# BIT-DYN/OpenObj

Measured on AMD Instinct MI355X. Metric: training rays/sec/GPU @64 samples/ray, 50 obj; PSNR delta vs ref, higher is better.
Workload: dtype f32; 1 GPU; c2: Replica room_0-shaped, 50 object MLPs on this GPU (hidden 32), 4096 rays/object/step, 64 samples/ray (16+48), RGB+depth+opacity loss, fused fwd+loss+bwd+AdamW; objects_per_gpu=50, objects_total=50, rays_per_object=4096, samples_per_ray=64, hidden=32, feature_head=False, background_mlp=True, parallelism=objects sharded x1, rccl_ranks=1, launched_by=single process, loss_status=0

## Files before the change

openobj_amd/csrc/objnerf_mlp32.h:

```cpp
#pragma once
#include "objnerf_mlp.h"

namespace obj32n {
using namespace obj32;

constexpr int WROW = 40;
constexpr int R_IN = 0;
constexpr int R_M1 = R_IN + 96;
constexpr int R_CAT = R_M1 + 32;
constexpr int R_M2 = R_CAT + 128;
constexpr int R_CL = R_M2 + 32;
constexpr int R_FL = R_CL + 80;
constexpr int ROWS_NOFEAT = R_FL, ROWS_FEAT = R_FL + 80;
constexpr int SV_BM1 = 0, SV_BM2 = 32, SV_WA = 64, SV_WOC = 96, SV_HB = 192, SV_PEB = 196, SV_FLOATS = 196 + 72 + 4;
__host__ __device__ constexpr int img_floats(bool feat) { return (feat ? ROWS_FEAT : ROWS_NOFEAT) * WROW + SV_FLOATS; }
__host__ __device__ constexpr int sv_base(bool feat) { return (feat ? ROWS_FEAT : ROWS_NOFEAT) * WROW; }

constexpr int BIAS_COL = -2, ZERO_COL = -1;
__host__ __device__ inline int x1_col(int t, int g) {
  const int i = t >> 2, f = t & 3, j = 4 * i + g;
  if (j < OBJ_NDIR) return 3 + OBJ_NDIR * f + j;
  if (f == 0) return g - 1;
  if (f == 1 && g == 1) return BIAS_COL;
  return ZERO_COL;
// ... 262 lines not shown
#pragma unroll
    for (int r = 0; r < 4; ++r) {
      const int col = x2_col(4 * T + r, g);
      e.x2[T][r] = col >= 0 ? emb[OBJ_E1 + col] : (col == BIAS_COL ? 1.0f : 0.0f);
    }
}

#ifdef OBJ_PRIO_TOGGLE
__device__ __forceinline__ void prio_layer(const int layer) {
  const int grp = __builtin_amdgcn_readfirstlane((int)(threadIdx.x >> 8)) & 1;
  if (layer >= 0 && ((layer ^ grp) & 1)) __builtin_amdgcn_s_setprio(1); else __builtin_amdgcn_s_setprio(0);
}
#else
__device__ __forceinline__ void prio_layer(const int) {}
#endif

template <bool FEAT>
__device__ __forceinline__ void mlp32_trunk(const float* wf, const float* sv, const int g, const Emb32& e, Acts& a) {
  T32 acc = zero32();
  prio_layer(1);
#pragma unroll
  for (int T = 0; T < 6; ++T) mma_f16(acc, wf, R_IN + 16 * T, e.x1[T]);
  a.h1 = relu32(acc);
  prio_layer(2);
#pragma unroll
  for (int tt = 0; tt < 2; ++tt)
#pragma unroll
    for (int r = 0; r < 4; ++r) acc.t[tt][r] = sv[SV_BM1 + 16 * tt + 4 * g + r];
  mma_f32(acc, wf, R_M1, a.h1);
  a.h2 = relu32(acc);
  prio_layer(3);
  acc = zero32();
  mma_f32(acc, wf, R_CAT, a.h2);
#pragma unroll
  for (int T = 0; T < 6; ++T) mma_f16(acc, wf, R_CAT + 32 + 16 * T, e.x1[T]);
  a.h3 = relu32(acc);
  prio_layer(4);
#pragma unroll
  for (int tt = 0; tt < 2; ++tt)
#pragma unroll
    for (int r = 0; r < 4; ++r) acc.t[tt][r] = sv[SV_BM2 + 16 * tt + 4 * g + r];
  mma_f32(acc, wf, R_M2, a.h3);
  a.h4 = relu32(acc);
  prio_layer(5);
  acc = zero32();
  mma_f32(acc, wf, R_CL, a.h4);
#pragma unroll
  for (int T = 0; T < 3; ++T) mma_f16(acc, wf, R_CL + 32 + 16 * T, e.x2[T]);
  a.hc = relu32(acc);
  if (FEAT) {
    acc = zero32();
    mma_f32(acc, wf, R_FL, a.h4);
#pragma unroll
    for (int T = 0; T < 3; ++T) mma_f16(acc, wf, R_FL + 32 + 16 * T, e.x2[T]);
    a.hf = relu32(acc);
  }
  prio_layer(-1);
}
__device__ __forceinline__ void mlp32_head_sums(const float* sv, const int g, const Acts& a, float& sa, float& s0, float& s1,
                                                float& s2) {
  float pa = 0.f, pc0 = 0.f, pc1 = 0.f, pc2 = 0.f;
#pragma unroll
  for (int tt = 0; tt < 2; ++tt)
#pragma unroll
    for (int r = 0; r < 4; ++r) {
      const int row = 16 * tt + 4 * g + r;
      pa = fmaf(sv[SV_WA + row], a.h4.t[tt][r], pa);
      pc0 = fmaf(sv[SV_WOC + row], a.hc.t[tt][r], pc0);
      pc1 = fmaf(sv[SV_WOC + H + row], a.hc.t[tt][r], pc1);
      pc2 = fmaf(sv[SV_WOC + 2 * H + row], a.hc.t[tt][r], pc2);
    }
  sa = xgroup_sum(pa); s0 = xgroup_sum(pc0); s1 = xgroup_sum(pc1); s2 = xgroup_sum(pc2);
}
template <bool FEAT>
__device__ __forceinline__ float mlp32_forward(const float* wf, const float* sv, const int g, const Emb32& e, Acts& a) {
  mlp32_trunk<FEAT>(wf, sv, g, e, a);
  float sa, s0, s1, s2;
  mlp32_head_sums(sv, g, a, sa, s0, s1, s2);
  const float mine = (g == 0) ? sa : ((g == 1) ? s0 : ((g == 2) ? s1 : s2));
  const float z = mine + sv[SV_HB + g];
  return (g == 0) ? z * 10.0f : sigmoid_acc(z);
}
template <bool FEAT>
__device__ __forceinline__ void mlp32_forward_all(const float* wf, const float* sv, const int g, const Emb32& e, Acts& a,
                                                  float& alpha10, float& colour) {
  mlp32_trunk<FEAT>(wf, sv, g, e, a);
  float sa, s0, s1, s2;
  mlp32_head_sums(sv, g, a, sa, s0, s1, s2);
  alpha10 = (sa + sv[SV_HB]) * 10.0f;
  const float mine = (g == 1) ? s0 : ((g == 2) ? s1 : s2);
  colour = (g == 0) ? 0.0f : sigmoid_acc(mine + sv[SV_HB + g]);
}

}
```

openobj_amd/csrc/objnerf_train32.hip:

```cpp
#include <mutex>
#include "objnerf_mlp32.h"
#include "objnerf_train_common.h"
#include "../../include/objnerf_hip.h"

using namespace obj32n;
using namespace objtrain;

#if !defined(OBJ_LAZY_HEADS) && !defined(OBJ_BUTTERFLY_HEADS)
#define OBJ_LAZY_HEADS
#endif

#ifndef OBJ32_ABL
#define OBJ32_ABL 0
#endif
#define TILE_SYNC() do { if (!((OBJ32_ABL) & 2)) __syncthreads(); } while (0)
#ifndef OBJ32_WG_UNROLL_FAST
#define OBJ32_WG_UNROLL_FAST 16
#endif

namespace {

__device__ __forceinline__ void st_T32(float* stg_lane, const int rowbase, const T32& v) {
  if ((OBJ32_ABL) & 4) { asm volatile("" :: "v"(v.t[0]), "v"(v.t[1])); return; }
#pragma unroll
// ... 23 lines not shown
    acc1 = OBJ_MFMA(a1[1], b[1], acc1);
  }
}

template <int UNR = 8>
__device__ __forceinline__ void wg_half(f32x4& acc0, const float* dT, const float* aT) {
  if ((OBJ32_ABL) & 8) return;
  dT = (const float*)__builtin_assume_aligned(dT, 8);
  aT = (const float*)__builtin_assume_aligned(aT, 8);
#pragma unroll UNR
  for (int st = 0; st < 32; st += 2) {
    const f32x2 b = *reinterpret_cast<const f32x2*>(aT + st);
    const f32x2 a0 = *reinterpret_cast<const f32x2*>(dT + st);
    acc0 = OBJ_MFMA(a0[0], b[0], acc0);
    acc0 = OBJ_MFMA(a0[1], b[1], acc0);
  }
}

template <int UNR = 8>
__device__ __forceinline__ void wg_quarter(f32x4& acc0, const float* dT, const float* aT, const int st0) {
  if ((OBJ32_ABL) & 8) return;
  dT = (const float*)__builtin_assume_aligned(dT, 8);
  aT = (const float*)__builtin_assume_aligned(aT, 8);
#pragma unroll UNR
  for (int st = st0; st < st0 + 16; st += 2) {
    const f32x2 b = *reinterpret_cast<const f32x2*>(aT + st);
    const f32x2 a0 = *reinterpret_cast<const f32x2*>(dT + st);
    acc0 = OBJ_MFMA(a0[0], b[0], acc0);
    acc0 = OBJ_MFMA(a0[1], b[1], acc0);
  }
}

__device__ __forceinline__ void wr_pair(float* slab, const f32x4& a0, const f32x4& a1, const int g, const int col,
                                        const int w_off, const int ncols, const int b_off) {
#pragma unroll
  for (int r = 0; r < 4; ++r) {
    const int o0 = 4 * g + r, o1 = 16 + 4 * g + r;
    if (col >= 0) {
      slab[w_off + o0 * ncols + col] = a0[r];
      slab[w_off + o1 * ncols + col] = a1[r];
    } else if (col == BIAS_COL && b_off >= 0) {
      slab[b_off + o0] = a0[r];
      slab[b_off + o1] = a1[r];
    }
  }
}

__device__ __forceinline__ void wr_half(float* slab, const f32x4& a0, const int half, const int g, const int col,
                                        const int w_off, const int ncols, const int b_off) {
#pragma unroll
  for (int r = 0; r < 4; ++r) {
    const int o = 16 * half + 4 * g + r;
    if (col >= 0) slab[w_off + o * ncols + col] = a0[r];
    else if (col == BIAS_COL && b_off >= 0) slab[b_off + o] = a0[r];
  }
}

#ifdef PHASE_TIMING
__device__ unsigned long long g_phase32[8][24];
#define PT_INIT() unsigned long long pt_acc[18]; for (int i_ = 0; i_ < 18; ++i_) pt_acc[i_] = 0; \
  unsigned long long pt_t0 = __builtin_amdgcn_s_memtime()
#define PT(i) do { const unsigned long long t_ = __builtin_amdgcn_s_memtime(); pt_acc[i] += t_ - pt_t0; pt_t0 = t_; } while (0)
#define PT_FLUSH() do { if (blockIdx.x == 0 && lane == 0) for (int i_ = 0; i_ < 18; ++i_) g_phase32[w][i_] = pt_acc[i_]; } while (0)
#else
#define PT_INIT() do {} while (0)
#define PT(i) do {} while (0)
#define PT_FLUSH() do {} while (0)
#endif

template <bool FEAT>
struct Lay {
  static constexpr int IMG = img_floats(FEAT);
  static constexpr int ROWS = FEAT ? 160 : STG_ROWS;
  static constexpr int LDS_FLOATS = IMG + SM_FLOATS + ROWS * STG_LD;
  static constexpr int A_H3 = FEAT ? 0 : 96, A_DHC = FEAT ? 80 : 128, A_DHF = 112, A_DH4 = FEAT ? 80 : 160;
  static constexpr int C_DH2 = FEAT ? 128 : 160;
  static_assert(LDS_FLOATS * 4 <= 163840, "LDS budget");
  static_assert((IMG * 4) % 16 == 0, "staging area alignment");
};
constexpr int F_SW = 144 * STG_LD;
constexpr int F_GFH = F_SW + TS;
constexpr int F_GOF = F_GFH + 16 * 32;
static_assert(F_GOF + 32 <= 160 * STG_LD && OFF_FHB + 64 * NWAVE <= 80 * STG_LD, "feature aliases");

template <bool FEAT, bool MASKS, int SS>
__global__ __launch_bounds__(NTHR) void train_fused32_kernel(const TrainDev a) {
  typedef Lay<FEAT> LY;
  constexpr int IMG = LY::IMG;
  constexpr bool FAST = !FEAT;
  constexpr int WGU = (!FEAT && !MASKS && SS == 64) ? OBJ32_WG_UNROLL_FAST : 8;
  extern __shared__ __attribute__((aligned(16))) float lds[];
  const int tid = threadIdx.x;
  const int lane = tid & 63;
  const int w = __builtin_amdgcn_readfirstlane(tid >> 6);
  const int c = lane & 15, g = lane >> 4;
  float* sv = lds + sv_base(FEAT);
  float* s_alpha = lds + IMG;
  float* s_col = s_alpha + TS;
  float* stg = lds + IMG + SM_FLOATS;

  const long T_flat = (long)a.K * a.NT;
  long cur = a.flat_nwg ? T_flat * blockIdx.x / a.flat_nwg : 0;
  const long cur_end = a.flat_nwg ? T_flat * (blockIdx.x + 1) / a.flat_nwg : 1;
  bool first_seg = true;
  while (cur < cur_end) {
  int k, t0, t1, tstep, sslot;
  if (a.flat_nwg) {
    k = (int)(cur / a.NT);
    t0 = (int)(cur - (long)k * a.NT);
    const long rem = cur_end - cur;
    t1 = (long)t0 + rem < (long)a.NT ? (int)(t0 + rem) : a.NT;
    tstep = 1;
    sslot = (int)blockIdx.x - flat_wg_of(T_flat, a.flat_nwg, (long)k * a.NT);
    cur += t1 - t0;
  } else {
    k = blockIdx.x / a.G; t0 = blockIdx.x % a.G; t1 = a.NT; tstep = a.G; sslot = t0;
    cur = cur_end;
  }
  const int n_slots = a.flat_nwg ? a.Gs : a.G;
  if (!first_seg) __syncthreads();
  first_seg = false;

  stage_weights32(lds, a.params + (long)k * a.p_stride, a.L, FEAT, tid, NTHR);
  for (int i = tid; i < LY::ROWS * STG_LD; i += NTHR) stg[i] = 0.0f;
  __syncthreads();

  const float scale = a.scale[k];
  const int S = SS ? SS : a.S, R = a.R, TR = SS ? TS / SS : a.TR;
  const float n1 = (float)a.counts[2 * k], n2 = (float)a.counts[2 * k + 1];
  int bflag0, bflag1;
  batch_flags(a, bflag0, bflag1);
  const float inv1 = bflag0 ? 0.0f : 1.0f / (n1 + 1e-10f);
  const float inv2 = bflag1 ? 0.0f : 1.0f / (n2 + 1e-10f);

  const float* wf = (const float*)__builtin_assume_aligned(lds + 4 * g * WROW + out_pos(c), 8);
  const float* wt0 = (const float*)__builtin_assume_aligned(lds + c * WROW + 8 * g + 4 * (g & 1), 16);
  const float* wt1 = (const float*)__builtin_assume_aligned(lds + c * WROW + 8 * g + 4 * (1 - (g & 1)), 16);
  float* stg_lane = stg + (4 * g) * STG_LD + 16 * w + c;
  const float* lane_rd = stg + c * STG_LD + 32 * g;

  f32x4 accA0 = zero4(), accA1 = zero4(), accB0 = zero4(), accB1 = zero4(), accC0 = zero4(), accC1 = zero4();
  f32x4 accA2 = zero4(), accC2 = zero4();
#ifdef OBJ_LAZY_HEADS
  constexpr bool LAZY_H = !FEAT;
#else
  constexpr bool LAZY_H = false;
#endif
  float hW[4][8];
#pragma unroll
  for (int s_ = 0; s_ < 8; ++s_) hW[0][s_] = hW[1][s_] = hW[2][s_] = hW[3][s_] = 0.f;
  float gS0 = 0.f;
  float gS1 = 0.f;
#ifdef OBJ_LAZY_BIAS
  float bS[2][8];
#pragma unroll
  for (int s_ = 0; s_ < 8; ++s_) bS[0][s_] = bS[1][s_] = 0.f;
#else
  float gS2 = 0.f;
#endif
  float g_hb = 0.f;
  float dB[6][3];
#pragma unroll
  for (int i = 0; i < 6; ++i) dB[i][0] = dB[i][1] = dB[i][2] = 0.f;
  float l_d = 0.f, l_c = 0.f, l_o = 0.f, l_f = 0.f;

  auto fetch_point = [&](const int tile_, const int slot_, float& x, float& y, float& z_) {
    const int q_ = slot_ / S, si_ = slot_ - q_ * S;
    const int ray_ = tile_ * TR + q_;
    x = 0.f; y = 0.f; z_ = 0.f;
    if (tile_ < t1 && q_ < TR && ray_ < a.R) {
      const long rr = (long)k * a.R + ray_;
      if (a.pts) {
        const float* p = a.pts + (rr * S + si_) * 3;
        x = p[0]; y = p[1]; z_ = p[2];
      } else {
        const float zz = a.z[rr * S + si_];
        const float* o = a.origins + rr * 3;
        const float* d = a.dirs + rr * 3;
        x = (o[0] + d[0] * zz) - a.obj_center;
        y = (o[1] + d[1] * zz) - a.obj_center;
        z_ = (o[2] + d[2] * zz) - a.obj_center;
      }
    }
  };
  const bool rows_mode = SS ? true : seg_is_rows(S);
  const SegRows seg_rows = SegRows::make(rows_mode ? S : 64, lane);
  const int slot = 16 * w + c;
  float nx, ny, nz;
  fetch_point(t0, slot, nx, ny, nz);
  PT_INIT();
  for (int tile = t0; tile < t1; tile += tstep) {
    asm volatile("" ::: "memory");
    const int ray0 = tile * TR;
    const int q = slot / S;
    const int ray = ray0 + q;
    const bool valid = (q < TR) && (ray < R);
    Pe32 pe;
    pe32_project(sv, g, nx, ny, nz, scale, pe);
    PT(0);
    Acts act;
    {
      Emb32 e;
      embed32(e, pe, g);
      PT(1);
      if (MASKS && a.emb_debug && valid) {
        float* er = a.emb_debug + (((long)k * R + ray) * S + (slot - q * S)) * (OBJ_E1 + OBJ_E2);
#pragma unroll
        for (int T_ = 0; T_ < 6; ++T_)
#pragma unroll
          for (int r_ = 0; r_ < 4; ++r_) {
            const int col = x1_col(4 * T_ + r_, g);
            if (col >= 0) er[col] = e.x1[T_][r_];
          }
#pragma unroll
        for (int T_ = 0; T_ < 3; ++T_)
#pragma unroll
          for (int r_ = 0; r_ < 4; ++r_) {
            const int col = x2_col(4 * T_ + r_, g);
            if (col >= 0) er[OBJ_E1 + col] = e.x2[T_][r_];
          }
      }
      s_alpha[g * TS + slot] = mlp32_forward<FEAT>(wf, sv, g, e, act);
    }
    if (MASKS && a.relu_masks) {
      uint8_t* dst = a.relu_masks + (((long)k * R + (valid ? ray : 0)) * S + (slot - q * S)) * 24;
      write_relu_mask(dst, 0, g, act.h1, valid);
      write_relu_mask(dst, 1, g, act.h2, valid);
      write_relu_mask(dst, 2, g, act.h3, valid);
      write_relu_mask(dst, 3, g, act.h4, valid);
      write_relu_mask(dst, 4, g, act.hc, valid);
      if (FEAT) write_relu_mask(dst, 5, g, act.hf, valid);
    }
    unsigned hf_pos = 0;
    if (FEAT) {
#pragma unroll
      for (int tt = 0; tt < 2; ++tt)
#pragma unroll
        for (int r = 0; r < 4; ++r) hf_pos |= (act.hf.t[tt][r] > 0.0f ? 1u : 0u) << (4 * tt + r);
#pragma unroll
      for (int tt = 0; tt < 2; ++tt)
#pragma unroll
        for (int r = 0; r < 4; ++r) stg[slot * HF_LD + 16 * tt + 4 * g + r] = act.hf.t[tt][r];
      for (int i = tid; i < 32 * 32 + 33; i += NTHR) {
        const float v = a.gram[(long)k * GRAM + i];
        if (i < 1024) stg[OFF_GBUF + (i >> 5) * 33 + (i & 31)] = v;
        else stg[OFF_GBUF + 32 * 33 + (i - 1024)] = v;
      }
    }
    PT(2);
    auto ray_inputs = [&](const int ps_, float& zz_, float& gtd_, float& gr_, float& gg_, float& gb_, int& lab_) {
      const int rpp_ = 64 / S;
      const int ql_ = lane / S, pos_ = lane - ql_ * S;
      const int qq_ = ps_ * rpp_ + ql_;
      const int rayq_ = ray0 + qq_;
      zz_ = 0.f; gtd_ = 0.f; gr_ = 0.f; gg_ = 0.f; gb_ = 0.f; lab_ = 2;
      if ((ql_ < rpp_) && (qq_ < TR) && (rayq_ < R)) {
        const long rr = (long)k * R + rayq_;
        zz_ = a.z[rr * S + pos_];
        gtd_ = a.gt_depth[rr];
        gr_ = a.gt_rgb[rr * 3]; gg_ = a.gt_rgb[rr * 3 + 1]; gb_ = a.gt_rgb[rr * 3 + 2];
        lab_ = a.labels[rr];
      }
    };
    float pf_zz = 0.f, pf_gtd = 0.f, pf_gr = 0.f, pf_gg = 0.f, pf_gb = 0.f;
    int pf_lab = 2;
    if (w * (64 / S) < TR) ray_inputs(w, pf_zz, pf_gtd, pf_gr, pf_gg, pf_gb, pf_lab);
    auto feat_inputs = [&](const int ps_, const int qb_, float& uh_, float& beta_, float& ngv_, int& lab_) {
      const int rpp_ = 64 / S;
      const int ql2_ = qb_ + (lane >> 5);
      const int qq2_ = ps_ * rpp_ + ql2_;
      const int ray2_ = ray0 + qq2_;
      uh_ = 0.f; beta_ = 0.f; ngv_ = 1.f; lab_ = 2;
      if ((ql2_ < rpp_) && (qq2_ < TR) && (ray2_ < R)) {
        const long rr2_ = (long)k * R + ray2_;
        uh_ = a.rayin[rr2_ * RAYIN + (lane & 31)];
        beta_ = a.rayin[rr2_ * RAYIN + 32];
        ngv_ = a.rayin[rr2_ * RAYIN + 33];
        lab_ = (int)a.labels[rr2_];
      }
    };
    float pf_uh = 0.f, pf_beta = 0.f, pf_ngv = 1.f;
    int pf_lab2 = 2;
    if (FEAT && S == 64) {
      if (valid) {
        const long rr2_ = (long)k * R + ray;
        pf_uh = a.rayin[rr2_ * RAYIN + (lane & 31)];
        pf_beta = a.rayin[rr2_ * RAYIN + 32];
        pf_ngv = a.rayin[rr2_ * RAYIN + 33];
        pf_lab2 = (int)a.labels[rr2_];
      }
    } else if (FEAT && w * (64 / S) < TR) feat_inputs(w, 0, pf_uh, pf_beta, pf_ngv, pf_lab2);
    TILE_SYNC();
    PT(3);
    auto composite_passes = [&](const auto& sg) {
      const int rpp = 64 / S;
      const int npass = (TR + rpp - 1) / rpp;
      for (int ps = w; ps < npass; ps += NWAVE) {
        const int ql = lane / S, pos = lane - ql * S;
        const int qq = ps * rpp + ql;
        const int rayq = ray0 + qq;
        const bool on = (ql < rpp) && (qq < TR) && (rayq < R);
        const int sl = qq * S + pos;
        float al = 0.f, c0 = 0.f, c1 = 0.f, c2 = 0.f, zz = pf_zz;
        float gtd = pf_gtd, gr = pf_gr, gg = pf_gg, gb = pf_gb;
        int lab = pf_lab;
        if (ps != w) ray_inputs(ps, zz, gtd, gr, gg, gb, lab);
        if (on) { al = s_alpha[sl]; c0 = s_col[sl]; c1 = s_col[TS + sl]; c2 = s_col[2 * TS + sl]; }
        const float occ = on ? sigmoid_acc(al) : 0.0f;
        const float fr = on ? (1.0f - occ) + 1e-10f : 1.0f;
        const float Pinc = sg.scan_mul(fr, pos);
        float T = __shfl_up(Pinc, 1, 64);
        if (pos == 0) T = 1.0f;
        const float wgt = occ * T;
        const float D = sg.total_add(wgt * zz, pos);
        const float O = sg.total_add(wgt, pos);
        const float C0 = sg.total_add(wgt * c0, pos);
        const float C1 = sg.total_add(wgt * c1, pos);
        const float C2 = sg.total_add(wgt * c2, pos);
        const float dz = zz - D;
        const float V = sg.total_add(wgt * (dz * dz), pos);
        const float m1 = (lab == 1) ? 1.0f : 0.0f;
        const float m2 = (lab != 2) ? 1.0f : 0.0f;
        const float tgt = (lab != 0) ? 1.0f : 0.0f;
        const float info = 1.0f / (sqrtf(V) + 1e-4f);
        const float rd = D - gtd, r0 = C0 - gr, r1 = C1 - gg, r2 = C2 - gb, ro = O - tgt;
        auto sgn = [](float x) { return x > 0.f ? 1.0f : (x < 0.f ? -1.0f : 0.0f); };
        const float gD = m1 * sgn(rd) * info * inv1;
        const float gC0 = a.color_scaling * m1 * sgn(r0) * inv1;
        const float gC1 = a.color_scaling * m1 * sgn(r1) * inv1;
        const float gC2 = a.color_scaling * m1 * sgn(r2) * inv1;
        const float gO = a.opacity_scaling * m2 * sgn(ro) * inv2;
        if (on && pos == 0) {
          l_d += m1 * fabsf(rd) * info * inv1;
          l_c += m1 * (fabsf(r0) + fabsf(r1) + fabsf(r2)) * inv1;
          l_o += m2 * fabsf(ro) * inv2;
        }
        float dw = gD * zz + gO + gC0 * c0 + gC1 * c1 + gC2 * c2;
        if (FEAT) {
          float* s_w = stg + F_SW;
          float* s_gfh = stg + F_GFH;
          float* s_gof = stg + F_GOF;
          float* s_fhb = stg + OFF_FHB + 64 * w;
          const float* Gb = stg + OFF_GBUF;
          if (on) s_w[sl] = wgt;
          if (on && pos == 0) s_gof[16 + qq] = O;
          __builtin_amdgcn_wave_barrier();
          asm volatile("" ::: "memory");
          const int half = lane >> 5, hh = lane & 31;
          for (int qb = 0; qb < rpp; qb += 2) {
            const int ql2 = qb + half;
            const int qq2 = ps * rpp + ql2;
            const int ray2 = ray0 + qq2;
            const bool on2 = (ql2 < rpp) && (qq2 < TR) && (ray2 < R);
            const long rr2 = (long)k * R + (on2 ? ray2 : 0);
            float fh = 0.f;
            if (rpp == 1) {
              const bool on1 = (qb < rpp) && (ps * rpp + qb < TR) && (ray0 + ps * rpp + qb < R);
              const int q1 = ps * rpp + qb;
              if (on1) {
                float f0 = 0.f, f1 = 0.f, f2 = 0.f, f3 = 0.f;
                const float* wp = s_w + q1 * S;
                const float* hp = stg + (q1 * S) * HF_LD + hh;
                int s2 = half;
                for (; s2 + 6 < S; s2 += 8) {
                  f0 = fmaf(wp[s2], hp[s2 * HF_LD], f0);
                  f1 = fmaf(wp[s2 + 2], hp[(s2 + 2) * HF_LD], f1);
                  f2 = fmaf(wp[s2 + 4], hp[(s2 + 4) * HF_LD], f2);
                  f3 = fmaf(wp[s2 + 6], hp[(s2 + 6) * HF_LD], f3);
                }
                for (; s2 < S; s2 += 2) f0 = fmaf(wp[s2], hp[s2 * HF_LD], f0);
                fh = (f0 + f1) + (f2 + f3);
              }
              fh += __shfl_xor(fh, 32, 64);
            } else if (on2) {
              for (int s2 = 0; s2 < S; ++s2) fh = fmaf(s_w[qq2 * S + s2], stg[(qq2 * S + s2) * HF_LD + hh], fh);
            }
// ... 92 lines not shown
          l_c += m1 * (fabsf(r0) + fabsf(r1) + fabsf(r2)) * inv1;
          l_o += m2 * fabsf(ro) * inv2;
          s_gof[16 + w] = O;
        }
        dw = gD * zz + gO + gC0 * c0 + gC1 * c1 + gC2 * c2;
        if (on) s_w[sl] = wgt;
      }
      TILE_SYNC();
      {
        const float wv = valid ? s_w[slot] : 0.0f;
        float v8[8];
#pragma unroll
        for (int tt = 0; tt < 2; ++tt)
#pragma unroll
          for (int r = 0; r < 4; ++r) v8[4 * tt + r] = wv * stg[slot * HF_LD + 16 * tt + 4 * g + r];
        const float psum = slot_sums8(v8, c);
        if (c < 8) s_part[w * 32 + 16 * ((c & 7) >> 2) + 4 * g + (c & 3)] = psum;
      }
      TILE_SYNC();
      {
        float* s_fhb = stg + OFF_FHB + 64 * w;
        const float* Gb = stg + OFF_GBUF;
        const int half = lane >> 5, hh = lane & 31;
        const int w0 = w & ~3;
        const float fh = valid ? (s_part[w0 * 32 + hh] + s_part[(w0 + 1) * 32 + hh]) +
                                 (s_part[(w0 + 2) * 32 + hh] + s_part[(w0 + 3) * 32 + hh]) : 0.0f;
        if (half == 0) s_fhb[hh] = fh;
        __builtin_amdgcn_wave_barrier();
        asm volatile("" ::: "memory");
        float Gp = 0.f;
#pragma unroll
        for (int h2 = 0; h2 < 16; ++h2) Gp = fmaf(Gb[hh * 33 + 16 * half + h2], s_fhb[16 * half + h2], Gp);
        const float Gfh = Gp + __shfl_xor(Gp, 32, 64);
        const float wbh = Gb[32 * 33 + hh], bb = Gb[32 * 33 + 32];
        const float uh = pf_uh, beta = pf_beta, ngv = pf_ngv;
        const float O2 = valid ? s_gof[16 + q] : 0.f;
        const float fu = wave_sum32(fh * uh), fGf = wave_sum32(fh * Gfh), fwb = wave_sum32(fh * wbh);
        const float dotFg = fu + O2 * beta;
        const float nF2 = fmaxf(fGf + 2.0f * O2 * fwb + O2 * O2 * bb, 0.0f);
        const float nF = fmaxf(sqrtf(nF2), 1e-8f), ngc = fmaxf(ngv, 1e-8f);
        const float cosv = dotFg / (nF * ngc);
        const float mm1 = (pf_lab2 == 1) ? 1.0f : 0.0f;
        const float gam = -a.feat_scaling * mm1 * inv1;
        const float ar = gam / (nF * ngc), cr = -gam * cosv / (nF * nF);
        const float gfh = ar * uh + cr * (Gfh + O2 * wbh);
        const float gof = ar * beta + cr * (fwb + O2 * bb);
        if (valid && (w & 3) == 0 && half == 0) {
          const long rr2 = (long)k * R + ray;
          if (hh == 0) {
            l_f += mm1 * (1.0f - cosv) * inv1;
            a.rayfeat[rr2 * RAYFEAT + 32] = O2;
            a.rayfeat[rr2 * RAYFEAT + 33] = ar;
            a.rayfeat[rr2 * RAYFEAT + 34] = cr;
          }
          s_gfh[q * 32 + hh] = gfh;
          a.rayfeat[rr2 * RAYFEAT + hh] = fh;
        }
        if (half == 0) s_fhb[32 + hh] = gfh;
        __builtin_amdgcn_wave_barrier();
        asm volatile("" ::: "memory");
        float dp = 0.f;
#pragma unroll
        for (int tt = 0; tt < 2; ++tt)
#pragma unroll
          for (int r = 0; r < 4; ++r)
            dp = fmaf(s_fhb[32 + 16 * tt + 4 * g + r], stg[slot * HF_LD + 16 * tt + 4 * g + r], dp);
        const float dwf = xgroup_sum(dp) + gof;
        if (g == 0 && valid) s_dwf[slot] = dwf;
      }
      TILE_SYNC();
      if (w < TR) {
        if (on) dw += s_dwf[sl];
        const float qv = dw * wgt;
        const float suf = sg.rscan_add(qv, pos) - qv;
        const float docc = dw * T - suf / fr;
        if (on) {
          s_alpha[sl] = 10.0f * (docc * occ * (1.0f - occ));
          s_col[sl] = gC0 * wgt * c0 * (1.0f - c0);
          s_col[TS + sl] = gC1 * wgt * c1 * (1.0f - c1);
          s_col[2 * TS + sl] = gC2 * wgt * c2 * (1.0f - c2);
        }
      }
    } else if ((OBJ32_ABL) & 1) {
    } else if (SS || rows_mode) composite_passes(seg_rows); else composite_passes(SegGeneric{S});
    PT(4);
    TILE_SYNC();
    PT(5);
    const float da = valid ? s_alpha[slot] : 0.0f;
    const float dc0 = valid ? s_col[slot] : 0.0f;
    const float dc1 = valid ? s_col[TS + slot] : 0.0f;
    const float dc2 = valid ? s_col[2 * TS + slot] : 0.0f;
    g_hb += (g == 0) ? da : ((g == 1) ? dc0 : ((g == 2) ? dc1 : dc2));
    float dps[6];
#pragma unroll
    for (int i = 0; i < 6; ++i) dps[i] = 0.f;
#pragma unroll
    for (int i = 0; i < 6; ++i) asm volatile("" : "+v"(pe.vh[i]), "+v"(pe.vl[i]));

    T32 d_hf = zero32();
    if (FEAT) {
      const float wv = valid ? stg[F_SW + slot] : 0.0f;
#pragma unroll
      for (int tt = 0; tt < 2; ++tt)
#pragma unroll
        for (int r = 0; r < 4; ++r) {
          const float gv = valid ? stg[F_GFH + q * 32 + 16 * tt + 4 * g + r] : 0.0f;
          d_hf.t[tt][r] = ((hf_pos >> (4 * tt + r)) & 1u) ? wv * gv : 0.0f;
        }
    }
    T32 d_hc, d_h4;
    float pa_[8];
    float pb_[8], pc_[8], pd_[8];
#pragma unroll
    for (int tt = 0; tt < 2; ++tt)
#pragma unroll
      for (int r = 0; r < 4; ++r) {
        const int row = 16 * tt + 4 * g + r;
        const int s = 4 * tt + r;
        const float hv = act.hc.t[tt][r];
        if (LAZY_H) {
          hW[0][s] = fmaf(da, act.h4.t[tt][r], hW[0][s]);
          hW[1][s] = fmaf(dc0, hv, hW[1][s]);
          hW[2][s] = fmaf(dc1, hv, hW[2][s]);
          hW[3][s] = fmaf(dc2, hv, hW[3][s]);
        } else {
          pa_[s] = da * act.h4.t[tt][r];
          pb_[s] = dc0 * hv;
          pc_[s] = dc1 * hv;
          pd_[s] = dc2 * hv;
        }
        const float dv = fmaf(sv[SV_WOC + 2 * H + row], dc2, fmaf(sv[SV_WOC + H + row], dc1, sv[SV_WOC + row] * dc0));
        d_hc.t[tt][r] = hv > 0.0f ? dv : 0.0f;
        d_h4.t[tt][r] = sv[SV_WA + row] * da;
      }
    if (!LAZY_H) {
      gS0 += slot_sums16(pa_, pb_, c);
      gS1 += slot_sums16(pc_, pd_, c);
      asm volatile("" : "+v"(gS0), "+v"(gS1));
    }
    st_T32(stg_lane, 0, act.h4);
    if (!FEAT) st_T32(stg_lane, LY::A_H3, act.h3);
    st_T32(stg_lane, LY::A_DHC, d_hc);
    if (FEAT) st_T32(stg_lane, LY::A_DHF, d_hf);
    mma_t32<FAST>(d_h4, wt0, wt1, R_CL, d_hc);
    if (FEAT) mma_t32<FAST>(d_h4, wt0, wt1, R_FL, d_hf);
    d_h4 = relu_mask32(d_h4, act.h4);
#ifdef OBJ_LAZY_BIAS
#pragma unroll
    for (int tt = 0; tt < 2; ++tt)
#pragma unroll
      for (int r = 0; r < 4; ++r) bS[1][4 * tt + r] += d_h4.t[tt][r];
#else
#pragma unroll
    for (int tt = 0; tt < 2; ++tt)
#pragma unroll
      for (int r = 0; r < 4; ++r) pa_[4 * tt + r] = d_h4.t[tt][r];
    {
      const float sv8 = slot_sums8(pa_, c);
      gS2 += (c >= 8) ? sv8 : 0.0f;
      asm volatile("" : "+v"(gS2));
    }
#endif
    if (!FEAT) st_T32(stg_lane, LY::A_DH4, d_h4);
#pragma unroll
    for (int T = 0; T < 3; ++T) {
      f32x4 d_x = zero4();
      mma_t16<FAST>(d_x, wt0, wt1, R_CL + 32 + 16 * T, d_hc);
      if (FEAT) mma_t16<FAST>(d_x, wt0, wt1, R_FL + 32 + 16 * T, d_hf);
      float o0, o1, o2, o3;
      pe32_x2_pair_fb(pe, 2 * T, g, d_x[0], d_x[1], dps[2 * T], o0, o1);
      pe32_x2_pair_fb(pe, 2 * T + 1, g, d_x[2], d_x[3], dps[2 * T + 1], o2, o3);
      st_T16(stg_lane, 32 + 16 * T, f32x4{o0, o1, o2, o3});
    }
    T32 d_h3 = zero32();
// ... 90 lines not shown
      wg_pair<WGU>(accC0, accC1, lane_rd + dTr * STG_LD, lane_rd + aTr * STG_LD);
    }
    PT(16);
    PT(17);
  }
  PT_FLUSH();

  float* slab = a.slab + ((long)k * n_slots + sslot) * a.slab_stride;
  const Layout& L = a.L;
  {
    int t_, g_;
    auto cl_col = [&](const int rho) {
      int col = rho;
      if (rho >= H) { kappa_tg(rho - H, t_, g_); col = x2_col(t_, g_); if (col >= 0) col += H; }
      return col;
    };
    if (FEAT) {
      if (w < 5) wr_pair(slab, accA0, accA1, g, cl_col(16 * w + c), L.cl_w, H + OBJ_E2, L.cl_b);
      else wr_pair(slab, accA0, accA1, g, cl_col(16 * (w - 5) + c), L.fl_w, H + OBJ_E2, L.fl_b);
      const int half = w & 1, t2 = (w & 3) >> 1;
      if (w < 4) wr_half(slab, accA2, half, g, cl_col(48 + 16 * t2 + c), L.fl_w, H + OBJ_E2, L.fl_b);
      else wr_half(slab, accA2, half, g, 16 * t2 + c, L.m2_w, H, -1);
    } else if (w < 5) {
      wr_pair(slab, accA0, accA1, g, cl_col(16 * w + c), L.cl_w, H + OBJ_E2, L.cl_b);
    } else if (w < 7) {
      wr_pair(slab, accA0, accA1, g, 16 * (w - 5) + c, L.m2_w, H, -1);
    }
    {
      const int rho = 16 * w + c;
      int col = rho;
      if (rho >= H) { kappa_tg(rho - H, t_, g_); col = x1_col(t_, g_); if (col >= 0) col += H; }
      wr_pair(slab, accB0, accB1, g, col, L.cat_w, H + OBJ_E1, L.cat_b);
    }
    if (w < 6) {
      kappa_tg(16 * w + c, t_, g_);
      wr_pair(slab, accC0, accC1, g, x1_col(t_, g_), L.in_w, OBJ_E1, L.in_b);
    } else if (!FEAT) {
      wr_pair(slab, accC0, accC1, g, 16 * (w - 6) + c, L.m1_w, H, -1);
    }
  }
  if (FEAT) {
    __syncthreads();
    float* xch = stg + (w >> 1) * 256 + 4 * lane;
    if (w & 1) *reinterpret_cast<f32x4*>(xch) = accC2;
    __syncthreads();
    if (!(w & 1)) {
      accC2 += *reinterpret_cast<const f32x4*>(xch);
      wr_half(slab, accC2, (w >> 1) & 1, g, 16 * (w >> 2) + c, L.m1_w, H, -1);
    }
  }
  __syncthreads();
  float* red = stg;
  constexpr int NRED32 = 6 * 32 + 4 + 4 + 72;
  {
    float* mine = red + w * NRED32;
    {
      const int s = c & 7;
      const int row = 16 * (s >> 2) + 4 * g + (s & 3);
      if (LAZY_H) {
#pragma unroll
        for (int s_ = 0; s_ < 8; ++s_) {
          const int rw = 16 * (s_ >> 2) + 4 * g + (s_ & 3);
          const float v2 = dpp_rowsum16(hW[0][s_]), v3 = dpp_rowsum16(hW[1][s_]);
          const float v4 = dpp_rowsum16(hW[2][s_]), v5 = dpp_rowsum16(hW[3][s_]);
          if (c == 0) { mine[64 + rw] = v2; mine[96 + rw] = v3; mine[128 + rw] = v4; mine[160 + rw] = v5; }
        }
      } else {
        if (c < 8) { mine[64 + row] = gS0; mine[128 + row] = gS1; }
        else { mine[96 + row] = gS0; mine[160 + row] = gS1; }
      }
#ifdef OBJ_LAZY_BIAS
#pragma unroll
      for (int s_ = 0; s_ < 8; ++s_) {
        const int rw = 16 * (s_ >> 2) + 4 * g + (s_ & 3);
        const float v0 = dpp_rowsum16(bS[0][s_]), v1 = dpp_rowsum16(bS[1][s_]);
        if (c == 0) { mine[rw] = v0; mine[32 + rw] = v1; }
      }
#else
      mine[(c < 8 ? 0 : 32) + row] = gS2;
#endif
    }
    const float hb = dpp_rowsum16(g_hb);
    if (c == 0) mine[192 + g] = hb;
    const float e0 = wave_sum64(l_d), e1 = wave_sum64(l_c), e2 = wave_sum64(l_o);
    const float e3 = FEAT ? wave_sum64(l_f) : 0.0f;
    if (lane == 0) { mine[196] = e0; mine[197] = e1; mine[198] = e2; mine[199] = e3; }
#pragma unroll
    for (int i = 0; i < 6; ++i)
#pragma unroll
      for (int x = 0; x < 3; ++x) {
        const float v = dpp_rowsum16(dB[i][x]);
        if (c == 0) mine[200 + 12 * i + 3 * g + x] = v;
      }
  }
  __syncthreads();
  for (int i = tid; i < NRED32; i += NTHR) {
    float v = 0.f;
#pragma unroll
    for (int ww = 0; ww < NWAVE; ++ww) v += red[ww * NRED32 + i];
    if (i < 32) slab[L.m1_b + i] = v;
    else if (i < 64) slab[L.m2_b + i - 32] = v;
    else if (i < 96) slab[L.a_w + i - 64] = v;
    else if (i < 192) slab[L.oc_w + i - 96] = v;
    else if (i == 192) slab[L.a_b] = v;
    else if (i < 196) slab[L.oc_b + i - 193] = v;
    else if (i < 200) a.loss_part[((long)k * n_slots + sslot) * 4 + (i - 196)] = v;
    else if (i - 200 < 3 * OBJ_NDIR) slab[L.pe_b + (i - 200)] = v;
  }
  }
}

}

namespace objtrain {

size_t fused32_lds_bytes() { return (size_t)Lay<false>::LDS_FLOATS * 4; }

void launch_train32(const TrainDev& d, void* stream, bool feat) {
  constexpr int n0 = Lay<false>::LDS_FLOATS * 4, n1 = Lay<true>::LDS_FLOATS * 4;
  objnerf_once_per_device([] {
    (void)hipFuncSetAttribute((const void*)train_fused32_kernel<false, false, 64>, hipFuncAttributeMaxDynamicSharedMemorySize, n0);
    (void)hipFuncSetAttribute((const void*)train_fused32_kernel<false, false, 0>, hipFuncAttributeMaxDynamicSharedMemorySize, n0);
    (void)hipFuncSetAttribute((const void*)train_fused32_kernel<false, true, 0>, hipFuncAttributeMaxDynamicSharedMemorySize, n0);
    (void)hipFuncSetAttribute((const void*)train_fused32_kernel<true, false, 0>, hipFuncAttributeMaxDynamicSharedMemorySize, n1);
    (void)hipFuncSetAttribute((const void*)train_fused32_kernel<true, false, 64>, hipFuncAttributeMaxDynamicSharedMemorySize, n1);
    (void)hipFuncSetAttribute((const void*)train_fused32_kernel<true, true, 0>, hipFuncAttributeMaxDynamicSharedMemorySize, n1);
  });
  const dim3 grid(d.flat_nwg ? d.flat_nwg : d.K * d.G), blk(NTHR);
  hipStream_t st = (hipStream_t)stream;
  if (feat) {
    if (d.relu_masks || d.emb_debug) hipLaunchKernelGGL((train_fused32_kernel<true, true, 0>), grid, blk, n1, st, d);
    else if (d.S == 64) hipLaunchKernelGGL((train_fused32_kernel<true, false, 64>), grid, blk, n1, st, d);
    else hipLaunchKernelGGL((train_fused32_kernel<true, false, 0>), grid, blk, n1, st, d);
  } else if (d.relu_masks || d.emb_debug) hipLaunchKernelGGL((train_fused32_kernel<false, true, 0>), grid, blk, n0, st, d);
  else if (d.S == 64) hipLaunchKernelGGL((train_fused32_kernel<false, false, 64>), grid, blk, n0, st, d);
  else hipLaunchKernelGGL((train_fused32_kernel<false, false, 0>), grid, blk, n0, st, d);
}

}

#ifdef PHASE_TIMING
extern "C" int objnerf_debug_phase32(unsigned long long* out_host) {
  if (hipDeviceSynchronize() != hipSuccess) return -1;
  return hipMemcpyFromSymbol(out_host, HIP_SYMBOL(g_phase32), sizeof(unsigned long long) * 8 * 24) == hipSuccess ? 0 : -1;
}
#endif
```

Baseline: 21.69 million rays/s.

## Composite 64-sample rays in registers via per-wave quarter records and cross-lane scans

For the fast path with 64 samples per ray and no feature head, each wave computes a local quarter of a ray's transmittance scan, weight sums and depth moments using permlane swaps and DPP ops. It writes a small per-wave record to LDS, and the four waves of a ray combine those records to form the ray-level loss and gradients. This replaces the LDS round-trip composite passes and removes one tile-wide barrier. The cost is more complex cross-lane code, a reworked loss accumulation, and possible numerical differences in the depth-variance term.

Measured after the change: 21.11 million rays/s (median of 2 runs). 0.973x the previous value.

```diff
diff --git a/openobj_amd/csrc/objnerf_mlp32.h b/openobj_amd/csrc/objnerf_mlp32.h
--- a/openobj_amd/csrc/objnerf_mlp32.h
+++ b/openobj_amd/csrc/objnerf_mlp32.h
@@ -368,6 +368,18 @@
   return (g == 0) ? z * 10.0f : sigmoid_acc(z);
 }
 template <bool FEAT>
+__device__ __forceinline__ float mlp32_forward_sel(const float* wf, const float* sv, const int g, const Emb32& e, Acts& a,
+                                                   const bool occ_head) {
+  mlp32_trunk<FEAT>(wf, sv, g, e, a);
+  float sa, s0, s1, s2;
+  mlp32_head_sums(sv, g, a, sa, s0, s1, s2);
+  const float mine = (g == 0) ? sa : ((g == 1) ? s0 : ((g == 2) ? s1 : s2));
+  const float z = mine + sv[SV_HB + g];
+  const float x = (g == 0) ? z * 10.0f : z;
+  const float s = sigmoid_acc(x);
+  return (g == 0 && !occ_head) ? x : s;
+}
+template <bool FEAT>
 __device__ __forceinline__ void mlp32_forward_all(const float* wf, const float* sv, const int g, const Emb32& e, Acts& a,
                                                   float& alpha10, float& colour) {
   mlp32_trunk<FEAT>(wf, sv, g, e, a);
diff --git a/openobj_amd/csrc/objnerf_train32.hip b/openobj_amd/csrc/objnerf_train32.hip
--- a/openobj_amd/csrc/objnerf_train32.hip
+++ b/openobj_amd/csrc/objnerf_train32.hip
@@ -129,6 +129,35 @@
 constexpr int F_GFH = F_SW + TS;
 constexpr int F_GOF = F_GFH + 16 * 32;
 static_assert(F_GOF + 32 <= 160 * STG_LD && OFF_FHB + 64 * NWAVE <= 80 * STG_LD, "feature aliases");
+
+constexpr int QREC = 16;
+struct QuarterFwd { float occ, c0, c1, c2, fr, T, u; };
+__device__ __forceinline__ void quarter_local(QuarterFwd& f, float* rec, const float head, const float zz, const bool valid,
+                                              const int g, const int lane) {
+  const unsigned hu = __float_as_uint(head);
+  const auto s16 = __builtin_amdgcn_permlane16_swap(hu, hu, false, false);
+  const auto ev = __builtin_amdgcn_permlane32_swap(s16[0], s16[0], false, false);
+  const auto od = __builtin_amdgcn_permlane32_swap(s16[1], s16[1], false, false);
+  f.occ = valid ? __uint_as_float(ev[0]) : 0.0f;
+  f.c0 = __uint_as_float(od[0]); f.c1 = __uint_as_float(ev[1]); f.c2 = __uint_as_float(od[1]);
+  f.fr = (1.0f - f.occ) + 1e-10f;
+  float P = f.fr;
+  P *= dpp_mov<0x111>(1.0f, P); P *= dpp_mov<0x112>(1.0f, P); P *= dpp_mov<0x114>(1.0f, P); P *= dpp_mov<0x118>(1.0f, P);
+  f.T = dpp_mov<0x111>(1.0f, P);
+  f.u = f.occ * f.T;
+  const float r1 = dpp_rowsum16(f.u * ((g == 0) ? 1.0f : head));
+  const float su = lane_bcast(r1, 0), sc0 = lane_bcast(r1, 16), sc1 = lane_bcast(r1, 32), sc2 = lane_bcast(r1, 48);
+  const float suz = lane_bcast(dpp_rowsum16(f.u * zz), 0);
+  const float cen = su > 1e-30f ? suz * __builtin_amdgcn_rcpf(su) : 0.0f;
+  const float dz = zz - cen;
+  const float r2 = dpp_rowsum16((f.u * dz) * ((g == 0) ? 1.0f : dz));
+  const float prod = lane_bcast(P, 15), m1 = lane_bcast(r2, 0), m2 = lane_bcast(r2, 16);
+  if (lane == 0) {
+    *reinterpret_cast<f32x4*>(rec) = f32x4{prod, su, suz, sc0};
+    *reinterpret_cast<f32x4*>(rec + 4) = f32x4{sc1, sc2, cen, m1};
+    rec[8] = m2;
+  }
+}
 
 template <bool FEAT, bool MASKS, int SS>
 __global__ __launch_bounds__(NTHR) void train_fused32_kernel(const TrainDev a) {
@@ -170,10 +199,12 @@
 
   stage_weights32(lds, a.params + (long)k * a.p_stride, a.L, FEAT, tid, NTHR);
   for (int i = tid; i < LY::ROWS * STG_LD; i += NTHR) stg[i] = 0.0f;
+  if (!FEAT && tid < NWAVE * QREC) s_alpha[tid] = 0.0f;
   __syncthreads();
 
   const float scale = a.scale[k];
   const int S = SS ? SS : a.S, R = a.R, TR = SS ? TS / SS : a.TR;
+  const bool quarters = !FEAT && S == 64;
   const float n1 = (float)a.counts[2 * k], n2 = (float)a.counts[2 * k + 1];
   int bflag0, bflag1;
   batch_flags(a, bflag0, bflag1);
@@ -210,6 +241,7 @@
 #pragma unroll
   for (int i = 0; i < 6; ++i) dB[i][0] = dB[i][1] = dB[i][2] = 0.f;
   float l_d = 0.f, l_c = 0.f, l_o = 0.f, l_f = 0.f;
+  float l_q = 0.f;
 
   auto fetch_point = [&](const int tile_, const int slot_, float& x, float& y, float& z_) {
     const int q_ = slot_ / S, si_ = slot_ - q_ * S;
@@ -242,10 +274,20 @@
     const int q = slot / S;
     const int ray = ray0 + q;
     const bool valid = (q < TR) && (ray < R);
+    const int qi = w & 3;
+    float q_z = 0.f, q_tgt = 0.f;
+    int q_lab = 2;
+    if (quarters && valid) {
+      const long rr = (long)k * R + ray;
+      q_z = a.z[rr * S + (slot - q * S)];
+      q_lab = a.labels[rr];
+      if (c >= 2 && c <= 5) q_tgt = (c == 2) ? a.gt_depth[rr] : a.gt_rgb[rr * 3 + (c - 3)];
+    }
     Pe32 pe;
     pe32_project(sv, g, nx, ny, nz, scale, pe);
     PT(0);
     Acts act;
+    float head = 0.f;
     {
       Emb32 e;
       embed32(e, pe, g);
@@ -267,8 +309,10 @@
             if (col >= 0) er[OBJ_E1 + col] = e.x2[T_][r_];
           }
       }
-      s_alpha[g * TS + slot] = mlp32_forward<FEAT>(wf, sv, g, e, act);
-    }
+      if (FEAT) s_alpha[g * TS + slot] = mlp32_forward<FEAT>(wf, sv, g, e, act);
+      else head = mlp32_forward_sel<FEAT>(wf, sv, g, e, act, quarters);
+    }
+    if (!FEAT && !quarters) s_alpha[g * TS + slot] = head;
     if (MASKS && a.relu_masks) {
       uint8_t* dst = a.relu_masks + (((long)k * R + (valid ? ray : 0)) * S + (slot - q * S)) * 24;
       write_relu_mask(dst, 0, g, act.h1, valid);
@@ -311,7 +355,7 @@
     };
     float pf_zz = 0.f, pf_gtd = 0.f, pf_gr = 0.f, pf_gg = 0.f, pf_gb = 0.f;
     int pf_lab = 2;
-    if (w * (64 / S) < TR) ray_inputs(w, pf_zz, pf_gtd, pf_gr, pf_gg, pf_gb, pf_lab);
+    if (!quarters && w * (64 / S) < TR) ray_inputs(w, pf_zz, pf_gtd, pf_gr, pf_gg, pf_gb, pf_lab);
     auto feat_inputs = [&](const int ps_, const int qb_, float& uh_, float& beta_, float& ngv_, int& lab_) {
       const int rpp_ = 64 / S;
       const int ql2_ = qb_ + (lane >> 5);
@@ -337,8 +381,11 @@
         pf_lab2 = (int)a.labels[rr2_];
       }
     } else if (FEAT && w * (64 / S) < TR) feat_inputs(w, 0, pf_uh, pf_beta, pf_ngv, pf_lab2);
+    QuarterFwd qf = {0.f, 0.f, 0.f, 0.f, 1.f, 1.f, 0.f};
+    if (quarters && !((OBJ32_ABL) & 1)) quarter_local(qf, s_alpha + w * QREC, head, q_z, valid, g, lane);
     TILE_SYNC();
     PT(3);
+    float da = 0.f, dc0 = 0.f, dc1 = 0.f, dc2 = 0.f;
     auto composite_passes = [&](const auto& sg) {
       const int rpp = 64 / S;
       const int npass = (TR + rpp - 1) / rpp;
@@ -597,14 +644,54 @@
         }
       }
     } else if ((OBJ32_ABL) & 1) {
+      da = dc0 = dc1 = dc2 = head;
+    } else if (quarters) {
+      const float rv = s_alpha[(w & ~3) * QREC + lane];
+      const float p0 = lane_bcast(rv, 0), p1 = lane_bcast(rv, 16), p2 = lane_bcast(rv, 32);
+      const float p01 = p0 * p1, p012 = p01 * p2;
+      const float T0g = (g == 0) ? 1.0f : ((g == 1) ? p0 : ((g == 2) ? p01 : p012));
+      const float T0q = (qi == 0) ? 1.0f : ((qi == 1) ? p0 : ((qi == 2) ? p01 : p012));
+      const float val = T0g * rv;
+      const float tot = xgroup_sum(val);
+      const float D = lane_bcast(tot, 2);
+      const float m1v = dpp_mov<0x111>(0.0f, rv), cenv = dpp_mov<0x112>(0.0f, rv), suv = dpp_mov<0x117>(0.0f, rv);
+      const float dcn = D - cenv;
+      const float vq = fmaf(dcn * dcn, suv, fmaf(-2.0f * dcn, m1v, rv));
+      const float V = fmaxf(lane_bcast(xgroup_sum(T0g * vq), 8), 0.0f);
+      const float info = 1.0f / (sqrtf(V) + 1e-4f);
+      const float m1 = (q_lab == 1) ? 1.0f : 0.0f;
+      const float m2 = (q_lab != 2) ? 1.0f : 0.0f;
+      const float tgo = (q_lab != 0) ? 1.0f : 0.0f;
+      const float a1 = m1 * inv1;
+      const float lw = (c == 1) ? m2 * inv2 : ((c == 2) ? a1 * info : ((c >= 3 && c <= 5) ? a1 : 0.0f));
+      const float lsc = (c == 1) ? a.opacity_scaling : ((c == 2) ? 1.0f : a.color_scaling);
+      const float res = tot - ((c == 1) ? tgo : q_tgt);
+      const float gco = ((res > 0.f ? 1.0f : (res < 0.f ? -1.0f : 0.0f)) * lw) * lsc;
+      if (qi == 0 && valid) l_q += fabsf(res) * lw;
+      const float gO = lane_bcast(gco, 1), gD = lane_bcast(gco, 2);
+      const float gC0 = lane_bcast(gco, 3), gC1 = lane_bcast(gco, 4), gC2 = lane_bcast(gco, 5);
+      const float srow = dpp_rowsum16(val * gco);
+      const float later = xgroup_sum((g > qi) ? srow : 0.0f);
+      const float wgt = T0q * qf.u;
+      const float dw = gD * q_z + gO + gC0 * qf.c0 + gC1 * qf.c1 + gC2 * qf.c2;
+      float rs = dw * wgt;
+      rs += dpp_mov<0x101>(0.0f, rs); rs += dpp_mov<0x102>(0.0f, rs); rs += dpp_mov<0x104>(0.0f, rs); rs += dpp_mov<0x108>(0.0f, rs);
+      const float suf = dpp_mov<0x101>(0.0f, rs) + later;
+      const float docc = dw * (T0q * qf.T) - suf / qf.fr;
+      da = 10.0f * (docc * qf.occ * (1.0f - qf.occ));
+      dc0 = gC0 * wgt * qf.c0 * (1.0f - qf.c0);
+      dc1 = gC1 * wgt * qf.c1 * (1.0f - qf.c1);
+      dc2 = gC2 * wgt * qf.c2 * (1.0f - qf.c2);
     } else if (SS || rows_mode) composite_passes(seg_rows); else composite_passes(SegGeneric{S});
     PT(4);
-    TILE_SYNC();
+    if (!quarters) {
+      TILE_SYNC();
+      da = valid ? s_alpha[slot] : 0.0f;
+      dc0 = valid ? s_col[slot] : 0.0f;
+      dc1 = valid ? s_col[TS + slot] : 0.0f;
+      dc2 = valid ? s_col[2 * TS + slot] : 0.0f;
+    }
     PT(5);
-    const float da = valid ? s_alpha[slot] : 0.0f;
-    const float dc0 = valid ? s_col[slot] : 0.0f;
-    const float dc1 = valid ? s_col[TS + slot] : 0.0f;
-    const float dc2 = valid ? s_col[2 * TS + slot] : 0.0f;
     g_hb += (g == 0) ? da : ((g == 1) ? dc0 : ((g == 2) ? dc1 : dc2));
     float dps[6];
 #pragma unroll
@@ -861,6 +948,11 @@
     }
     const float hb = dpp_rowsum16(g_hb);
     if (c == 0) mine[192 + g] = hb;
+    if (quarters) {
+      l_o = (lane == 1) ? l_q : 0.0f;
+      l_d = (lane == 2) ? l_q : 0.0f;
+      l_c = (lane >= 3 && lane <= 5) ? l_q : 0.0f;
+    }
     const float e0 = wave_sum64(l_d), e1 = wave_sum64(l_c), e2 = wave_sum64(l_o);
     const float e3 = FEAT ? wave_sum64(l_f) : 0.0f;
     if (lane == 0) { mine[196] = e0; mine[197] = e1; mine[198] = e2; mine[199] = e3; }
```
